# zhexin1904/gtsam_personal

Hardware: AMD Instinct MI355X
Metric: LM iterations/sec (higher is better)
Workload: dtype f64; 1 GPU; synthetic BAL 1000 cameras / 100000 points / 1000002 factors (GeneralSFMFactor<Cal3Bundler> + 2 priors), seed 42, METIS ordering (Ordering::Metis of the reference, fixture-carried permutation), LM legacy defaults; ordering=metis, cameras=1000, points=100000, factors=1000002, fronts=100001, parallelism=single GPU

## Files before the change

### gtsam_personal_amd/csrc/kernels_dense.hpp

```cpp
#pragma once
#include <hip/hip_runtime.h>

#include <type_traits>

#include "kernels_front.hpp"

namespace lmgpu {

typedef double double4_t __attribute__((ext_vector_type(4)));

struct RowSrc {
  int32_t idx;
  int32_t i;
};
__device__ __forceinline__ void assemble_row_body(const FrontDesc& F, int64_t f_off, int ld, const int32_t* __restrict__ rowptr, const RowSrc* __restrict__ src,
                                                  const ChildRef* __restrict__ childs, const int32_t* __restrict__ cmap,
                                                  const FrontFac* __restrict__ ffac, const FacDesc* __restrict__ fd, double* __restrict__ pool,
                                                  int R, bool with_factors) {
  const int lane = threadIdx.x & 63;
  double* Arow = pool + f_off + (size_t)R * ld;
  for (int e = rowptr[R]; e < rowptr[R + 1]; e++) {
    const RowSrc sr = src[e];
    if (sr.idx >= 0) {
      const ChildRef c = childs[sr.idx];
// ... 449 lines not shown
__global__ __launch_bounds__(256) void hbm_backsolve_dataflow_kernel(FrontDesc F, int64_t f_off, int ld, const int32_t* __restrict__ fxoff,
                                                                      const double* __restrict__ pool, const double* __restrict__ inv,
                                                                      const double* __restrict__ y, double* __restrict__ xbuf,
                                                                      unsigned int* __restrict__ flags, double* __restrict__ delta,
                                                                      int* __restrict__ status) {
  __shared__ double acc[NB];
  __shared__ double xs[NB];
  __shared__ int ok, s_ticket;
  const int nblk = gridDim.x;
  if (threadIdx.x == 0) s_ticket = (int)atomicAdd(&flags[nblk], 1u);
  __syncthreads();
  const int b = nblk - 1 - s_ticket;
  const int r0 = b * NB, nb = min(NB, F.nf - r0);
  const int tid = threadIdx.x, row = tid >> 2, quarter = tid & 3;
  const double* A = pool + f_off;
  if (tid < NB) acc[tid] = (tid < nb) ? y[r0 + tid] : 0.0;
  if (tid == 0) ok = 1;
  __syncthreads();
  const double* arow = A + (size_t)(r0 + row) * ld;
  double ibv[16];
  {
    const double* ib = inv + (size_t)b * NB * NB + row * NB + quarter * 16;
#pragma unroll
    for (int k = 0; k < 16; k++) ibv[k] = ib[k];
  }
  auto load_rv = [&](int j, double(&r)[16]) {
    const int c0 = j * NB, ncol = min(NB, F.nf - c0);
#pragma unroll
    for (int k = 0; k < 16; k++) {
      const int c = quarter * 16 + k;
      r[k] = (j > b && row < nb && c < ncol) ? arow[c0 + c] : 0.0;
    }
  };
  double rv[16], rv_next[16];
  load_rv(nblk - 1, rv);
  for (int j = nblk - 1; j > b; j--) {
    const int c0 = j * NB, ncol = min(NB, F.nf - c0);
    if (tid < NB) {
      double v = 0.0;
      if (tid < ncol) {
        long spins = 0;
        for (;;) {
          v = __hip_atomic_load(&xbuf[c0 + tid], __ATOMIC_RELAXED, __HIP_MEMORY_SCOPE_AGENT);
          if (__double_as_longlong(v) != -1LL) break;
          __builtin_amdgcn_s_sleep(1);
          if (++spins > 2000000L) {
            ok = 0;
            v = 0.0;
            break;
          }
        }
      }
      xs[tid] = v;
    }
    load_rv(j - 1, rv_next);
    __syncthreads();
    if (!ok) break;
    double s = 0;
#pragma unroll
    for (int k = 0; k < 16; k++) s += rv[k] * xs[quarter * 16 + k];
    s += __shfl_xor(s, 1);
    s += __shfl_xor(s, 2);
    if (quarter == 0) acc[row] -= s;
#pragma unroll
    for (int k = 0; k < 16; k++) rv[k] = rv_next[k];
    __syncthreads();
  }
  if (!ok) {
    if (tid == 0) atomicExch(status + 1, 1 + F.id);
  }
  double s = 0;
#pragma unroll
  for (int k = 0; k < 16; k++) s += ibv[k] * acc[quarter * 16 + k];
  s += __shfl_xor(s, 1);
  s += __shfl_xor(s, 2);
  if (quarter == 0 && row < nb) {
    const double pub = (s != s) ? __longlong_as_double(0x7ff8000000000000LL) : s;
    __hip_atomic_store(&xbuf[r0 + row], pub, __ATOMIC_RELAXED, __HIP_MEMORY_SCOPE_AGENT);
    delta[fxoff[F.fx_begin + r0 + row]] = s;
    if (s != s) atomicMin(status, F.id);
  }
}

__global__ __launch_bounds__(256) void hbm_backsolve_dataflow2_kernel(FrontDesc F, int64_t f_off, int ld, const int32_t* __restrict__ fxoff,
                                                                       const double* __restrict__ pool, const double* __restrict__ inv16,
                                                                       const double* __restrict__ y ,
                                                                       double* __restrict__ xbuf, unsigned int* __restrict__ flags,
                                                                       double* __restrict__ delta, int* __restrict__ status) {
  typedef double d4_t __attribute__((ext_vector_type(4)));
  constexpr int NB = 64;
  __shared__ double Rl[64][65];
  __shared__ double Xl[64][65];
  __shared__ double Ml[64][65];
  __shared__ double Il[4][16][17];
  __shared__ double acc[NB], xs[NB], ub[NB];
  __shared__ int ok, s_ticket;
  const int nblk = gridDim.x;
  if (threadIdx.x == 0) s_ticket = (int)atomicAdd(&flags[nblk], 1u);
  __syncthreads();
  const int b = nblk - 1 - s_ticket;
  const int r0 = b * NB, nb = min(NB, F.nf - r0);
  const int tid = threadIdx.x, row = tid >> 2, quarter = tid & 3, lane = tid & 63, wave = tid >> 6;
  const int kk = lane >> 4, cc = lane & 15;
  const double* A = pool + f_off;
  const int n = F.n;
  if (tid < NB) acc[tid] = (tid < nb) ? (y ? y[r0 + tid] : A[(size_t)(r0 + tid) * ld + n - 1]) : 0.0;
  if (tid == 0) ok = 1;
  for (int idx = tid; idx < 64 * 64; idx += 256) {
    const int p = idx >> 6, q = idx & 63;
    double v = (p == q) ? 1.0 : 0.0;
    if (p < nb && q < nb && q >= p) v = A[(size_t)(r0 + p) * ld + r0 + q];
    Rl[p][q] = v;
    Xl[p][q] = 0.0;
  }
  const double* I16 = inv16 + (size_t)(b >> 2) * 4096 + (size_t)(4 * (b & 3)) * 256;
  for (int idx = tid; idx < 4 * 256; idx += 256) Il[idx >> 8][(idx >> 4) & 15][idx & 15] = I16[idx];
  __syncthreads();
  if (wave == 0) {
#pragma unroll
    for (int h = 0; h < 4; h++) {
#pragma unroll
      for (int r = 0; r < 4; r++) Xl[16 * h + kk + 4 * r][16 * h + cc] = Il[h][kk + 4 * r][cc];
      __builtin_amdgcn_wave_barrier();
      asm volatile("s_waitcnt lgkmcnt(0)" ::: "memory");
#pragma unroll
      for (int g = h - 1; g >= 0; g--) {
        d4_t m = d4_t{0, 0, 0, 0};
#pragma unroll
        for (int k = g + 1; k <= h; k++)
#pragma unroll
          for (int r = 0; r < 4; r++) m = __builtin_amdgcn_mfma_f64_16x16x4f64(Rl[16 * g + cc][16 * k + 4 * r + kk], Xl[16 * k + 4 * r + kk][16 * h + cc], m, 0, 0, 0);
        d4_t x = d4_t{0, 0, 0, 0};
#pragma unroll
        for (int r = 0; r < 4; r++) x = __builtin_amdgcn_mfma_f64_16x16x4f64(-Il[g][cc][4 * r + kk], m[r], x, 0, 0, 0);
#pragma unroll
        for (int r = 0; r < 4; r++) Xl[16 * g + kk + 4 * r][16 * h + cc] = x[r];
        __builtin_amdgcn_wave_barrier();
        asm volatile("s_waitcnt lgkmcnt(0)" ::: "memory");
      }
    }
  }
  __syncthreads();
  if (b + 1 < nblk) {
    const int c0n = (b + 1) * NB, ncoln = min(NB, F.nf - c0n);
    for (int idx = tid; idx < 64 * 64; idx += 256) {
      const int p = idx >> 6, q = idx & 63;
      Rl[p][q] = (p < nb && q < ncoln) ? A[(size_t)(r0 + p) * ld + c0n + q] : 0.0;
    }
    __syncthreads();
#pragma unroll
    for (int h = 0; h < 4; h++) {
      d4_t m = d4_t{0, 0, 0, 0};
#pragma unroll
      for (int k = 0; k < 16; k++) m = __builtin_amdgcn_mfma_f64_16x16x4f64(Xl[16 * wave + cc][4 * k + kk], Rl[4 * k + kk][16 * h + cc], m, 0, 0, 0);
#pragma unroll
      for (int r = 0; r < 4; r++) Ml[16 * wave + kk + 4 * r][16 * h + cc] = m[r];
    }
  }
  __syncthreads();
  double ibv[16], mv[16];
#pragma unroll
  for (int k = 0; k < 16; k++) {
    ibv[k] = Xl[row][quarter * 16 + k];
    mv[k] = Ml[row][quarter * 16 + k];
  }
  const double* arow = A + (size_t)(r0 + row) * ld;
  auto load_rv = [&](int j, double(&r)[16]) {
    const int c0 = j * NB, ncol = min(NB, F.nf - c0);
#pragma unroll
    for (int k = 0; k < 16; k++) {
      const int c = quarter * 16 + k;
      r[k] = (j > b + 1 && row < nb && c < ncol) ? arow[c0 + c] : 0.0;
    }
  };
  auto poll = [&](int j) {
    const int c0 = j * NB, ncol = min(NB, F.nf - c0);
    if (tid < NB) {
      double v = 0.0;
      if (tid < ncol) {
        long spins = 0;
        for (;;) {
          v = __hip_atomic_load(&xbuf[c0 + tid], __ATOMIC_RELAXED, __HIP_MEMORY_SCOPE_AGENT);
          if (__double_as_longlong(v) != -1LL) break;
          __builtin_amdgcn_s_sleep(1);
          if (++spins > 2000000L) {
            ok = 0;
            v = 0.0;
            break;
          }
        }
      }
      xs[tid] = v;
    }
  };
  double rv[16], rv_next[16];
  load_rv(nblk - 1, rv);
  for (int j = nblk - 1; j > b + 1; j--) {
    poll(j);
    load_rv(j - 1, rv_next);
    __syncthreads();
    if (!ok) break;
    double s = 0;
#pragma unroll
    for (int k = 0; k < 16; k++) s += rv[k] * xs[quarter * 16 + k];
    s += __shfl_xor(s, 1);
    s += __shfl_xor(s, 2);
    if (quarter == 0) acc[row] -= s;
#pragma unroll
    for (int k = 0; k < 16; k++) rv[k] = rv_next[k];
    __syncthreads();
  }
  {
    double s = 0;
#pragma unroll
    for (int k = 0; k < 16; k++) s += ibv[k] * acc[quarter * 16 + k];
    s += __shfl_xor(s, 1);
    s += __shfl_xor(s, 2);
    if (quarter == 0) ub[row] = s;
  }
  double xr;
  if (b + 1 < nblk && ok) {
    poll(b + 1);
    __syncthreads();
    double s = 0;
#pragma unroll
    for (int k = 0; k < 16; k++) s += mv[k] * xs[quarter * 16 + k];
    s += __shfl_xor(s, 1);
    s += __shfl_xor(s, 2);
    xr = ub[row] - s;
  } else {
    __syncthreads();
    xr = ub[row];
  }
  if (!ok && tid == 0) atomicExch(status + 1, 1 + F.id);
  if (quarter == 0 && row < nb) {
    const double pub = (xr != xr) ? __longlong_as_double(0x7ff8000000000000LL) : xr;
    __hip_atomic_store(&xbuf[r0 + row], pub, __ATOMIC_RELAXED, __HIP_MEMORY_SCOPE_AGENT);
    delta[fxoff[F.fx_begin + r0 + row]] = xr;
    if (xr != xr) atomicMin(status, F.id);
  }
}

}
```

### gtsam_personal_amd/csrc/lmgpu.hip

```cpp
#include <hip/hip_runtime.h>
#include <rccl/rccl.h>

#include <algorithm>
#include <chrono>
#include <cmath>
#include <cstdio>
#include <cstdlib>
#include <cstring>
#include <condition_variable>
#include <limits>
#include <mutex>
#include <string>
#include <map>
#include <vector>

#include "../../include/lmgpu.h"
#include "kernels_dense.hpp"
#include "kernels_potrf.hpp"
#include "kernels_step.hpp"
#include "dense_schedule.hpp"
#include "kernels_batched.hpp"
#include "kernels_level.hpp"
#include "kernels_bayes.hpp"
#include "kernels_schur.hpp"
// ... 947 lines not shown
  if (h->cfg.world_size > 1) HIPCHECK(hipMemsetAsync(h->delta, 0, h->ntot * sizeof(double), s));
  const bool merge = h->merge_backsub && h->cfg.world_size == 1 && !(h->cfg.flags & LMGPU_FLAG_SPLIT_ROOT);
  const bool no_bsd_runs = dev_switch("LMGPU_NO_BSD_RUNS") != nullptr;
  const int NFR = (int)h->h_fronts.size();
  if (h->n_fill_backsub < 0 || h->fill_backsub_merge != (int)merge) {
    std::vector<FillChunk> fills;
    if (merge) {
      add_fill(fills, h->d_bs_done, (size_t)(NFR + h->levels.size() + 1) * sizeof(unsigned int), 0u);
      add_fill(fills, h->delta, h->ntot * sizeof(double), 0xffffffffu);
    }
    if (h->bsd_x_count > 0) {
      add_fill(fills, h->d_bsd_x, h->bsd_x_count * sizeof(double), 0xffffffffu);
      add_fill(fills, h->d_bsd_ticket, h->levels.size() * sizeof(unsigned int), 0u);
    }
    if (h->d_fill_backsub) {
      HIPCHECK(hipStreamSynchronize(s));
      (void)hipFree(h->d_fill_backsub);
      h->d_fill_backsub = nullptr;
    }
    h->n_fill_backsub = (int)fills.size();
    h->fill_backsub_merge = (int)merge;
    if (!fills.empty()) {
      const int rcu = upload(h, &h->d_fill_backsub, fills);
      if (rcu) return rcu;
    }
  }
  if (h->n_fill_backsub > 0) hipLaunchKernelGGL(fill_chunks_kernel, dim3(h->n_fill_backsub), dim3(256), 0, s, (const FillChunk*)h->d_fill_backsub);
  int seg_hi = -1, seg_lo = -1;
  auto run_level = [&](const LevelWork& L) {
    if (L.lds_nf_max > LDSB_SMALL_NF) {
      hipLaunchKernelGGL(lds_backsub_wide_kernel, dim3(L.list_count), dim3(256), (size_t)(L.lds_rsd_max + LDSB_TAIL) * sizeof(double), s,
                         (const int32_t*)(h->d_lists + L.list_begin), L.list_count, (const FrontDesc*)h->d_fronts, (const int32_t*)h->d_fxoff,
                         (const int32_t*)h->d_sxoff, (const double*)h->pool, h->delta, h->d_status);
    } else {
      hipLaunchKernelGGL(lds_backsub_kernel, dim3((L.list_count + 3) / 4), dim3(256), 0, s, (const int32_t*)(h->d_lists + L.list_begin),
                         L.list_count, (const FrontDesc*)h->d_fronts, (const int32_t*)h->d_fxoff, (const int32_t*)h->d_sxoff,
                         (const double*)h->pool, h->delta, h->d_status);
    }
  };
  auto flush_segment = [&]() -> int {
    if (seg_hi < 0) return LMGPU_OK;
    const int kt = h->kt.begin(LMGPU_KT_BACKSUB_LDS, s);
    if (seg_hi == seg_lo) {
      run_level(h->levels[seg_hi]);
    } else {
      const int b = h->levels[seg_lo].list_begin, e = h->levels[seg_hi].list_begin + h->levels[seg_hi].list_count;
      int rsdmax = 0;
      for (int l = seg_lo; l <= seg_hi; l++) rsdmax = std::max(rsdmax, h->levels[l].lds_rsd_max);
      hipLaunchKernelGGL(lds_backsub_merged_kernel, dim3(e - b), dim3(256), (size_t)(rsdmax + LDSB_TAIL) * sizeof(double), s, (const int32_t*)h->d_lists, b, e,
                         (const FrontDesc*)h->d_fronts, (const int32_t*)h->d_fxoff, (const int32_t*)h->d_sxoff, (const double*)h->pool, h->delta,
                         h->d_status, (const int32_t*)h->d_bs_parent, (const int32_t*)h->d_bs_pos, h->d_bs_done, h->d_bs_done + NFR + seg_hi);
    }
    h->kt.end(kt, s);
    seg_hi = seg_lo = -1;
    return LMGPU_OK;
  };
  for (int li = (int)h->levels.size() - 1; li >= 0; li--) {
    const LevelWork& L = h->levels[li];
    if (merge && !L.hbm.empty()) {
      const int rcf = flush_segment();
      if (rcf) return rcf;
    }
    const int brun = (merge && !h->bsd_run_of.empty() && !no_bsd_runs) ? h->bsd_run_of[li] : -1;
    if (brun >= 0) {
      const lmgpu_handle::BsdRun& R = h->bsd_runs[brun];
      const int kt = h->kt.begin(LMGPU_KT_BACKSUB_HBM, s);
      hipLaunchKernelGGL(hbm_backsolve_blocks_kernel, dim3(R.count), dim3(256), 0, s, (const BsdBlock*)(h->d_bsd_run_table + R.begin), h->d_bsd_ticket + li,
                         (const int32_t*)h->d_fxoff, (const int32_t*)h->d_sxoff, (const double*)h->pool, h->delta, h->d_bsd_x, h->d_status, 1);
      h->kt.end(kt, s);
    }
    if (L.bsd_count > 0 && brun == -1) {
      const int kt = h->kt.begin(LMGPU_KT_BACKSUB_HBM, s);
      hipLaunchKernelGGL(hbm_backsolve_blocks_kernel, dim3(L.bsd_count), dim3(256), 0, s, (const BsdBlock*)(h->d_bsd_table + L.bsd_begin),
                         (L.bsd_count <= h->num_cus && !h->bsd_ticket) ? (unsigned int*)nullptr : h->d_bsd_ticket + li, (const int32_t*)h->d_fxoff,
                         (const int32_t*)h->d_sxoff, (const double*)h->pool, h->delta, h->d_bsd_x, h->d_status);
      h->kt.end(kt, s);
    }
    for (int fi : L.hbm) {
      const FrontDesc& F = h->h_fronts[fi];
      if (F.nf <= BSS_MAX_NF) continue;
      const int64_t off = h->f_off[fi];
      const int ld = h->f_ld[fi];
      const int kt = h->kt.begin(LMGPU_KT_BACKSUB_HBM, s);
      const int nblk = (F.nf + NB - 1) / NB;
      const bool has_sep = F.n - F.nf - 1 > 0;
      if (has_sep)
        hipLaunchKernelGGL(hbm_rhs_init_kernel, dim3(F.nf), dim3(64), 0, s, F, off, ld, (const int32_t*)h->d_sxoff, (const double*)h->pool,
                           (const double*)h->delta, h->ywork);
      HIPCHECK(hipMemsetAsync(h->bs_flags, 0, (nblk + 1) * sizeof(unsigned int), s));
      HIPCHECK(hipMemsetAsync(h->bs_x, 0xff, (size_t)nblk * NB * sizeof(double), s));
      if (h->inv16_owner == fi && !dev_switch("LMGPU_NO_INV16_REUSE")) {
        hipLaunchKernelGGL(hbm_backsolve_dataflow2_kernel, dim3(nblk), dim3(256), 0, s, F, off, ld, (const int32_t*)h->d_fxoff, (const double*)h->pool,
                           (const double*)h->inv16, has_sep ? (const double*)h->ywork : (const double*)nullptr, h->bs_x, h->bs_flags, h->delta,
                           h->d_status);
      } else {
        if (!has_sep)
          hipLaunchKernelGGL(hbm_rhs_init_kernel, dim3(F.nf), dim3(64), 0, s, F, off, ld, (const int32_t*)h->d_sxoff, (const double*)h->pool,
                             (const double*)h->delta, h->ywork);
        hipLaunchKernelGGL((hbm_invert_diag_kernel<NB>), dim3(nblk), dim3(NB), 0, s, (const double*)(h->pool + off), ld, F.nf, h->bs_inv);
        hipLaunchKernelGGL((hbm_backsolve_dataflow_kernel<NB>), dim3(nblk), dim3(256), 0, s, F, off, ld, (const int32_t*)h->d_fxoff,
                           (const double*)h->pool, (const double*)h->bs_inv, (const double*)h->ywork, h->bs_x, h->bs_flags, h->delta,
                           h->d_status);
      }
      h->kt.end(kt, s);
    }
    if (merge) {
      if (L.list_count > 0) {
        if (seg_hi < 0) seg_hi = li;
        seg_lo = li;
      }
      if (li == 0 || !h->levels[li - 1].hbm.empty()) {
        const int rcf = flush_segment();
        if (rcf) return rcf;
      }
    } else if (L.list_count > 0) {
      const int kt = h->kt.begin(LMGPU_KT_BACKSUB_LDS, s);
      run_level(L);
      h->kt.end(kt, s);
    }
  }
  HIPCHECK(hipGetLastError());
  return LMGPU_OK;
}

__global__ void set_scalar_kernel(double* p, double v) { *p = v; }


int pcg_ensure(lmgpu_handle* h) {
  if (h->pcg_ready) return LMGPU_OK;
  const Plan& P = h->plan;
  std::vector<int32_t> xo(P.xoff.begin(), P.xoff.begin() + P.n_vars + 1);
  std::vector<int64_t> loff(P.n_vars);
  int64_t lsz = 0;
  for (int s = 0; s < P.n_vars; s++) {
    loff[s] = lsz;
    lsz += (int64_t)P.dims[s] * P.dims[s];
  }
  std::vector<FacDesc> fd(h->nfac);
  HIPCHECK(hipMemcpy(fd.data(), h->d_fd, fd.size() * sizeof(FacDesc), hipMemcpyDeviceToHost));
  std::vector<int64_t> yoff(h->nfac);
  int64_t ysz = 0;
  for (int f = 0; f < h->nfac; f++) {
    yoff[f] = ysz;
    ysz += fd[f].rows;
  }
  int rc;
  if ((rc = upload(h, &h->pcg_xoff, xo))) return rc;
  if ((rc = upload(h, &h->pcg_loff, loff))) return rc;
  if ((rc = upload(h, &h->pcg_yoff, yoff))) return rc;
  const size_t n = std::max(1, h->ntot);
  HIPCHECK(hipMalloc((void**)&h->pcg_H, std::max<int64_t>(1, lsz) * sizeof(double)));
  HIPCHECK(hipMalloc((void**)&h->pcg_L, std::max<int64_t>(1, lsz) * sizeof(double)));
  HIPCHECK(hipMalloc((void**)&h->pcg_rhs, n * sizeof(double)));
  HIPCHECK(hipMalloc((void**)&h->pcg_r, n * sizeof(double)));
  HIPCHECK(hipMalloc((void**)&h->pcg_p, n * sizeof(double)));
  HIPCHECK(hipMalloc((void**)&h->pcg_q, n * sizeof(double)));
  HIPCHECK(hipMalloc((void**)&h->pcg_y, std::max<int64_t>(1, ysz) * sizeof(double)));
  HIPCHECK(hipMalloc((void**)&h->pcg_part, 3 * PCG_MAXPART * sizeof(double)));
  HIPCHECK(hipMalloc((void**)&h->pcg_ctl, sizeof(PcgCtl)));
  HIPCHECK(hipHostMalloc((void**)&h->h_pcg_ctl, sizeof(PcgCtl), hipHostMallocDefault));
  HIPCHECK(hipHostMalloc((void**)&h->h_pcg_done, sizeof(int32_t), hipHostMallocDefault));
  for (int i = 0; i < 3; i++) HIPCHECK(hipEventCreate(&h->pcg_ev[i]));
  h->pcg_ready = true;
  return LMGPU_OK;
}

__global__ void pcg_reset_ctl_kernel(PcgCtl* c) {
  c->status = 0x7fffffff;
  c->iters = 0;
}

int pcg_solve_enqueue(lmgpu_handle* h, double lambda) {
  int rc = pcg_ensure(h);
  if (rc) return rc;
  const lmgpu_pcg_params& pp = h->pcgp;
  if (pp.maxIterations + 1 > h->pcg_cap) {
    if (h->pcg_gam) (void)hipFree(h->pcg_gam);
// ... 1478 lines not shown
        const FrontDesc& F = h->h_fronts[fi];
        const lmgpu_handle::GatherRange& G = h->gather[fi];
        if (fr.nf > NBO || (F.pad & 1) || G.leaf_count > 0 || G.pblk_short + G.pblk_long + G.vblk_count > 0 || dev_switch("LMGPU_NO_MED")) continue;
        med.push_back(fi);
        h->is_med[fi] = 1;
        L.med_max_fac = std::max(L.med_max_fac, F.fac_count);
        L.med_max_child = std::max(L.med_max_child, F.child_count);
        L.med_max_nf = std::max(L.med_max_nf, fr.nf);
        L.med_max_cols = std::max(L.med_max_cols, fr.n - fr.nf);
        L.med_max_n = std::max(L.med_max_n, (int)fr.n);
      }
      L.med_count = (int)med.size() - L.med_begin;
      max_med = std::max(max_med, L.med_count);
    }
    if ((rc = upload(h, &h->d_med_list, med))) return rc;
    if (max_med > 0) HIPCHECK(hipMalloc((void**)&h->inv16_med, (size_t)max_med * 16 * 256 * sizeof(double)));
    if ((rc = upload(h, &h->d_f_off, h->f_off))) return rc;
    if ((rc = upload(h, &h->d_f_ld, h->f_ld))) return rc;
  }
  if ((rc = upload(h, &h->d_row_begin, h->row_begin))) return rc;
  {
    std::vector<MedFront> mfs;
    for (const LevelWork& L : h->levels)
      for (int fi : L.hbm)
        if (h->is_med[fi]) mfs.push_back(MedFront{h->h_fronts[fi], h->f_off[fi], h->f_ld[fi], h->row_begin[fi]});
    if ((rc = upload(h, &h->d_med_fronts, mfs))) return rc;
    h->fuse_levels = (int)h->levels.size() >= 12 && h->cfg.world_size == 1;
    if (const char* e = dev_switch("LMGPU_FUSE_LEVELS")) h->fuse_levels = atoi(e) != 0 && h->cfg.world_size == 1;
    std::vector<LevelTask> tasks;
    int li = 0;
    for (LevelWork& L : h->levels) {
      const int l = li++;
      L.fuse_task_count = 0;
      int nmax, jcap, threads;
      if (!h->fuse_levels || L.med_count == 0 || !(L.med_max_fac > 0 || L.med_max_child > 0)) continue;
      if (h->merge_elim && h->elim_seg_of[l] != -1) continue;
      if (!level_lds_class(h, l, &nmax, &jcap, &threads)) continue;
      L.fuse_task_begin = (int)tasks.size();
      L.fuse_nmax = nmax;
      L.fuse_jcap = jcap;
      L.fuse_threads = 256;
      if (const char* e = dev_switch("LMGPU_FUSE_THREADS")) L.fuse_threads = atoi(e) == 1024 && threads == 1024 ? 1024 : 256;
      for (int q = 0; q < L.list_count; q++) tasks.push_back(LevelTask{0, L.list_begin + q, 0, 0});
      for (int m = 0; m < L.med_count; m++) {
        const FrontDesc& F = mfs[L.med_begin + m].F;
        for (int r = 0; r < F.n; r += 4) tasks.push_back(LevelTask{1, m, r, 0});
      }
      for (int m = 0; m < L.med_count; m++) tasks.push_back(LevelTask{2, m, 0, 0});
      for (int m = 0; m < L.med_count; m++) {
        const FrontDesc& F = mfs[L.med_begin + m].F;
        for (int st = 0; st * 64 < F.n - F.nf; st++) tasks.push_back(LevelTask{3, m, st, 0});
      }
      for (int m = 0; m < L.med_count; m++) {
        const FrontDesc& F = mfs[L.med_begin + m].F;
        const int S = (F.n - F.nf + 63) / 64;
        for (int sj = 0; sj < S; sj++)
          for (int si = 0; si <= sj; si++)
            for (int qd = 0; qd < 4; qd++) tasks.push_back(LevelTask{4, m, si | (sj << 8), qd});
      }
      L.fuse_task_count = (int)tasks.size() - L.fuse_task_begin;
    }
    if (!tasks.empty()) {
      if ((rc = upload(h, &h->d_level_tasks, tasks))) return rc;
      h->n_level_sync = (int)mfs.size();
      HIPCHECK(hipMalloc((void**)&h->d_level_sync, std::max<size_t>(1, mfs.size()) * sizeof(LevelSync)));
    } else {
      h->fuse_levels = false;
    }
  }
  if ((rc = upload(h, &h->d_rowptr, rowptr))) return rc;
  if ((rc = upload(h, &h->d_rowsrc, rowsrc))) return rc;
  if ((rc = upload(h, &h->d_gpblk, gpblk))) return rc;
  if ((rc = upload(h, &h->d_gzero, gzero))) return rc;
  if ((rc = upload(h, &h->d_gpent, gpent))) return rc;
  if ((rc = upload(h, &h->d_gvblk, gvblk))) return rc;
  if ((rc = upload(h, &h->d_gvent, gvent))) return rc;
  HIPCHECK(hipMalloc((void**)&h->d_gcorner, std::max<size_t>(1, (size_t)n_gleaf) * sizeof(double)));
  if ((rc = finalize_vectors(h))) return rc;
  {
    int max_nf = 1;
    for (int fi = 0; fi < NF; fi++)
      if (h->front_active[fi] && P.fronts[fi].cls == 1) max_nf = std::max(max_nf, P.fronts[fi].nf);
    const int max_blk = (max_nf + NB - 1) / NB;
    HIPCHECK(hipMalloc((void**)&h->bs_inv, (size_t)max_blk * NB * NB * sizeof(double)));
    HIPCHECK(hipMalloc((void**)&h->inv16, (size_t)((P.max_front_n + NBO - 1) / NBO + 2) * 16 * 256 * sizeof(double)));
    h->pflags_panels = (P.max_front_n + NBO - 1) / NBO + 1;
    HIPCHECK(hipMalloc((void**)&h->d_pflags, (size_t)h->pflags_panels * PDF_FLAG_WORDS * sizeof(unsigned int)));

    HIPCHECK(hipMalloc((void**)&h->bs_x, (size_t)max_blk * NB * sizeof(double)));
    HIPCHECK(hipMalloc((void**)&h->bs_flags, (size_t)(max_blk + 1) * sizeof(unsigned int)));
  }
  return LMGPU_OK;
}

int lmgpu_total_dim(const lmgpu_handle* h) { return (h && h->finalized) ? h->ntot : -1; }
int lmgpu_total_store(const lmgpu_handle* h) { return (h && h->finalized) ? h->nstore : -1; }

int lmgpu_set_values(lmgpu_handle* h, const double* packed) {
  if (!h) return LMGPU_INVALID;
  if (!h->finalized || !packed) {
    h->err = "lmgpu_set_values: refused (!h->finalized || !packed)";
    return LMGPU_INVALID;
  }
  int rc = need_device(h);
  if (rc) return rc;
  const Plan& P = h->plan;
  for (int t = 0; t < kNumVarTypes; t++) {
    if (P.type_count[t] == 0) continue;
    std::vector<double> buf((size_t)P.type_count[t] * kVarStore[t]);
    for (int s = 0; s < P.n_vars; s++)
      if (P.types[s] == t) std::memcpy(&buf[(size_t)P.tidx[s] * kVarStore[t]], packed + P.voff[s], kVarStore[t] * sizeof(double));
    HIPCHECK(hipMemcpy(h->vals[h->cur][t], buf.data(), buf.size() * sizeof(double), hipMemcpyHostToDevice));
  }
  h->have_values = true;
  return LMGPU_OK;
}

int lmgpu_get_values(lmgpu_handle* h, double* packed) {
  if (!h) return LMGPU_INVALID;
  if (!h->finalized || !packed || !h->have_values) {
    h->err = "lmgpu_get_values: refused (!h->finalized || !packed || !h->have_values)";
    return LMGPU_INVALID;
  }
  int rc = need_device(h);
  if (rc) return rc;
  const Plan& P = h->plan;
  HIPCHECK(hipStreamSynchronize(h->stream));
  for (int t = 0; t < kNumVarTypes; t++) {
    if (P.type_count[t] == 0) continue;
    std::vector<double> buf((size_t)P.type_count[t] * kVarStore[t]);
    HIPCHECK(hipMemcpy(buf.data(), h->vals[h->cur][t], buf.size() * sizeof(double), hipMemcpyDeviceToHost));
    for (int s = 0; s < P.n_vars; s++)
      if (P.types[s] == t) std::memcpy(packed + P.voff[s], &buf[(size_t)P.tidx[s] * kVarStore[t]], kVarStore[t] * sizeof(double));
  }
  return LMGPU_OK;
}

int lmgpu_save_values(lmgpu_handle* h) {
  if (!h) return LMGPU_INVALID;
  if (!h->finalized || !h->have_values) {
    h->err = "lmgpu_save_values: refused (!h->finalized || !h->have_values)";
    return LMGPU_INVALID;
  }
  int rc = need_device(h);
  if (rc) return rc;
  for (int t = 0; t < kNumVarTypes; t++) {
    const size_t bytes = std::max<size_t>(1, (size_t)h->plan.type_count[t] * kVarStore[t]) * sizeof(double);
    if (!h->saved[t]) HIPCHECK(hipMalloc((void**)&h->saved[t], bytes));
    HIPCHECK(hipMemcpyAsync(h->saved[t], h->vals[h->cur][t], bytes, hipMemcpyDeviceToDevice, h->stream));
  }
  HIPCHECK(hipStreamSynchronize(h->stream));
  return LMGPU_OK;
}

int lmgpu_restore_values(lmgpu_handle* h) {
  if (!h) return LMGPU_INVALID;
  if (!h->finalized || !h->saved[0]) {
    h->err = "lmgpu_restore_values: refused (!h->finalized || !h->saved[0])";
    return LMGPU_INVALID;
  }
  int rc = need_device(h);
  if (rc) return rc;
  for (int t = 0; t < kNumVarTypes; t++) {
    const size_t bytes = std::max<size_t>(1, (size_t)h->plan.type_count[t] * kVarStore[t]) * sizeof(double);
    HIPCHECK(hipMemcpyAsync(h->vals[h->cur][t], h->saved[t], bytes, hipMemcpyDeviceToDevice, h->stream));
  }
  return LMGPU_OK;
}

int lmgpu_error(lmgpu_handle* h, double* total) {
  if (!h) return LMGPU_INVALID;
  if (!h->finalized || !total || !h->have_values) {
// ... 1217 lines not shown
```

Measured before the change: 131.2 LM iterations/s.

## Add wide 128-row dataflow back-solve kernel for large HBM fronts

Replaces the 64-row-per-block dataflow back-substitution for large fronts with a 512-thread kernel that handles 128-row blocks. Each block inverts its two 64x64 diagonal sub-blocks with MFMA from reused inv16 inverses, precomputes the product with the next block's off-diagonal coupling and parks it in scratch, and then streams the remaining tiles with double-buffered loads while polling for upstream solutions. The aim is to halve the length of the serial dependency chain and take the coupling GEMV off the critical path. The cost is more registers and shared memory per block and a spin-limit fallback. The old kernel is now compiled only under test hooks.

```diff
diff --git a/gtsam_personal_amd/csrc/kernels_dense.hpp b/gtsam_personal_amd/csrc/kernels_dense.hpp
--- a/gtsam_personal_amd/csrc/kernels_dense.hpp
+++ b/gtsam_personal_amd/csrc/kernels_dense.hpp
@@ -555,11 +555,14 @@
   }
 }
 
+#ifdef LMGPU_TEST_HOOKS
+template <bool STAMP = false>
 __global__ __launch_bounds__(256) void hbm_backsolve_dataflow2_kernel(FrontDesc F, int64_t f_off, int ld, const int32_t* __restrict__ fxoff,
                                                                        const double* __restrict__ pool, const double* __restrict__ inv16,
                                                                        const double* __restrict__ y ,
                                                                        double* __restrict__ xbuf, unsigned int* __restrict__ flags,
-                                                                       double* __restrict__ delta, int* __restrict__ status) {
+                                                                       double* __restrict__ delta, int* __restrict__ status,
+                                                                       unsigned long long* __restrict__ stamps = nullptr) {
   typedef double d4_t __attribute__((ext_vector_type(4)));
   constexpr int NB = 64;
   __shared__ double Rl[64][65];
@@ -575,6 +578,7 @@
   const int r0 = b * NB, nb = min(NB, F.nf - r0);
   const int tid = threadIdx.x, row = tid >> 2, quarter = tid & 3, lane = tid & 63, wave = tid >> 6;
   const int kk = lane >> 4, cc = lane & 15;
+  if (STAMP && tid == 0) stamps[3 * b] = wall_clock64();
   const double* A = pool + f_off;
   const int n = F.n;
   if (tid < NB) acc[tid] = (tid < nb) ? (y ? y[r0 + tid] : A[(size_t)(r0 + tid) * ld + n - 1]) : 0.0;
@@ -694,6 +698,7 @@
   double xr;
   if (b + 1 < nblk && ok) {
     poll(b + 1);
+    if (STAMP && tid == 0) stamps[3 * b + 1] = wall_clock64();
     __syncthreads();
     double s = 0;
 #pragma unroll
@@ -712,6 +717,298 @@
     delta[fxoff[F.fx_begin + r0 + row]] = xr;
     if (xr != xr) atomicMin(status, F.id);
   }
-}
-
-}
+  if (STAMP && tid == 0) stamps[3 * b + 2] = wall_clock64();
+}
+#endif
+
+__device__ __forceinline__ void bsw_invert64(const double (*Rl)[65], double (*Xl)[65], const double (*Il)[16][17], int kk, int cc) {
+  typedef double d4_t __attribute__((ext_vector_type(4)));
+#pragma unroll
+  for (int h = 0; h < 4; h++) {
+#pragma unroll
+    for (int r = 0; r < 4; r++) Xl[16 * h + kk + 4 * r][16 * h + cc] = Il[h][kk + 4 * r][cc];
+    __builtin_amdgcn_wave_barrier();
+    asm volatile("s_waitcnt lgkmcnt(0)" ::: "memory");
+#pragma unroll
+    for (int g = h - 1; g >= 0; g--) {
+      d4_t m = d4_t{0, 0, 0, 0};
+#pragma unroll
+      for (int k = g + 1; k <= h; k++)
+#pragma unroll
+        for (int r = 0; r < 4; r++) m = __builtin_amdgcn_mfma_f64_16x16x4f64(Rl[16 * g + cc][16 * k + 4 * r + kk], Xl[16 * k + 4 * r + kk][16 * h + cc], m, 0, 0, 0);
+      d4_t x = d4_t{0, 0, 0, 0};
+#pragma unroll
+      for (int r = 0; r < 4; r++) x = __builtin_amdgcn_mfma_f64_16x16x4f64(-Il[g][cc][4 * r + kk], m[r], x, 0, 0, 0);
+#pragma unroll
+      for (int r = 0; r < 4; r++) Xl[16 * g + kk + 4 * r][16 * h + cc] = x[r];
+      __builtin_amdgcn_wave_barrier();
+      asm volatile("s_waitcnt lgkmcnt(0)" ::: "memory");
+    }
+  }
+}
+
+#define BSW_NB 128
+#define BSW_SPIN_LIMIT 2000000L
+template <bool STAMP = false>
+__global__ __launch_bounds__(512) void hbm_backsolve_wide_kernel(FrontDesc F, int64_t f_off, int ld, const int32_t* __restrict__ fxoff,
+                                                                  const double* __restrict__ pool, const double* __restrict__ inv16,
+                                                                  const double* __restrict__ y ,
+                                                                  double* __restrict__ xbuf, unsigned int* __restrict__ flags,
+                                                                  double* __restrict__ delta, int* __restrict__ status,
+                                                                  double* mpark ,
+                                                                  unsigned long long* __restrict__ stamps = nullptr) {
+  typedef double d4_t __attribute__((ext_vector_type(4)));
+  constexpr int NB = BSW_NB;
+  __shared__ double T[4][64][65];
+  __shared__ double Il[8][16][17];
+  __shared__ double rhs[NB], ub[NB];
+  __shared__ double xs[8][NB];
+  __shared__ int s_ticket;
+  const int nblk = gridDim.x;
+  if (threadIdx.x == 0) s_ticket = (int)atomicAdd(&flags[nblk], 1u);
+  __syncthreads();
+  const int b = nblk - 1 - s_ticket;
+  const int nf = F.nf, n = F.n;
+  const int r0 = b * NB, nb = min(NB, nf - r0);
+  const int tid = threadIdx.x, lane = tid & 63, wave = __builtin_amdgcn_readfirstlane(tid >> 6);
+  const int kk = lane >> 4, cc = lane & 15;
+  const double* A = pool + f_off;
+  if (STAMP && tid == 0) stamps[3 * b] = wall_clock64();
+  const int myslot = ((lane >> 5) & 1) * 8 + ((lane >> 4) & 1) * 4 + ((lane >> 3) & 1) * 2 + ((lane >> 2) & 1);
+  const int frow = 16 * wave + myslot;
+  const int frc = min(r0 + frow, nf - 1);
+  const double yv = y ? y[frc] : A[(size_t)frc * ld + n - 1];
+  const int hr = 2 * ((cc >> 3) & 1) + ((cc >> 2) & 1);
+  const int prow = 16 * wave + kk + 4 * hr;
+  const int po = fxoff[F.fx_begin + min(r0 + prow, nf - 1)];
+  const bool has_next = b + 1 < nblk;
+  const int c0n = (b + 1) * NB, ncoln = has_next ? min(NB, nf - c0n) : 0;
+  double g11[8], g22[8], g12[8], gn[2][2][8];
+#pragma unroll
+  for (int i = 0; i < 8; i++) {
+    const int p = wave + 8 * i, q = lane;
+    const double e = (p == q) ? 1.0 : 0.0;
+    g11[i] = (p < nb && q < nb && q >= p) ? A[(size_t)(r0 + p) * ld + r0 + q] : e;
+    g22[i] = (64 + p < nb && 64 + q < nb && q >= p) ? A[(size_t)(r0 + 64 + p) * ld + r0 + 64 + q] : e;
+    g12[i] = (p < nb && 64 + q < nb) ? A[(size_t)(r0 + p) * ld + r0 + 64 + q] : 0.0;
+#pragma unroll
+    for (int kh = 0; kh < 2; kh++)
+#pragma unroll
+      for (int ch = 0; ch < 2; ch++)
+        gn[kh][ch][i] = (64 * kh + p < nb && 64 * ch + q < ncoln) ? A[(size_t)(r0 + 64 * kh + p) * ld + c0n + 64 * ch + q] : 0.0;
+  }
+#pragma unroll
+  for (int i = 0; i < 8; i++) {
+    const int p = wave + 8 * i, q = lane;
+    T[0][p][q] = g11[i];
+    T[1][p][q] = g22[i];
+    T[2][p][q] = 0.0;
+    T[3][p][q] = 0.0;
+  }
+  const double* I16 = inv16 + (size_t)(b >> 1) * 4096 + (size_t)(8 * (b & 1)) * 256;
+  for (int idx = tid; idx < 8 * 256; idx += 512) {
+    const int h = idx >> 8, i = (idx >> 4) & 15, j = idx & 15;
+    Il[h][i][j] = (16 * h < nb) ? I16[idx] : ((i == j) ? 1.0 : 0.0);
+  }
+  __syncthreads();
+  if (wave < 2) bsw_invert64(T[wave], T[2 + wave], Il + 4 * wave, kk, cc);
+  __syncthreads();
+#pragma unroll
+  for (int i = 0; i < 8; i++) T[0][wave + 8 * i][lane] = g12[i];
+  __syncthreads();
+  {
+    const int ti = wave >> 1;
+#pragma unroll
+    for (int u = 0; u < 2; u++) {
+      const int tj = 2 * (wave & 1) + u;
+      d4_t m = d4_t{0, 0, 0, 0};
+#pragma unroll
+      for (int k = 0; k < 16; k++) m = __builtin_amdgcn_mfma_f64_16x16x4f64(T[0][16 * ti + cc][4 * k + kk], T[3][4 * k + kk][16 * tj + cc], m, 0, 0, 0);
+#pragma unroll
+      for (int r = 0; r < 4; r++) T[1][16 * ti + kk + 4 * r][16 * tj + cc] = m[r];
+    }
+    __syncthreads();
+#pragma unroll
+    for (int u = 0; u < 2; u++) {
+      const int tj = 2 * (wave & 1) + u;
+      d4_t m = d4_t{0, 0, 0, 0};
+#pragma unroll
+      for (int k = 0; k < 16; k++) m = __builtin_amdgcn_mfma_f64_16x16x4f64(-T[2][16 * ti + cc][4 * k + kk], T[1][4 * k + kk][16 * tj + cc], m, 0, 0, 0);
+#pragma unroll
+      for (int r = 0; r < 4; r++) T[0][16 * ti + kk + 4 * r][16 * tj + cc] = m[r];
+    }
+    __syncthreads();
+  }
+  d4_t mB[8];
+#pragma unroll
+  for (int h = 0; h < 8; h++) mB[h] = d4_t{0, 0, 0, 0};
+  if (has_next) {
+#pragma unroll
+    for (int kh = 0; kh < 2; kh++) {
+#pragma unroll
+      for (int ch = 0; ch < 2; ch++) {
+#pragma unroll
+        for (int i = 0; i < 8; i++) T[1][wave + 8 * i][lane] = gn[kh][ch][i];
+        __syncthreads();
+        if (wave < 4 || kh == 1) {
+          const double(*Xop)[65] = (wave >= 4) ? T[3] : (kh == 0 ? T[2] : T[0]);
+          const int xr0 = 16 * (wave & 3);
+#pragma unroll
+          for (int hh = 0; hh < 4; hh++)
+#pragma unroll
+            for (int k = 0; k < 16; k++)
+              mB[4 * ch + hh] = __builtin_amdgcn_mfma_f64_16x16x4f64(Xop[xr0 + cc][4 * k + kk], T[1][4 * k + kk][16 * hh + cc], mB[4 * ch + hh], 0, 0, 0);
+        }
+        __syncthreads();
+      }
+    }
+  }
+  double* Mp = mpark + (size_t)b * NB * NB + tid;
+  if (has_next) {
+#pragma unroll
+    for (int h = 0; h < 8; h++)
+#pragma unroll
+      for (int r = 0; r < 4; r++) Mp[(4 * h + r) * 512] = mB[h][r];
+  }
+  auto load_tile = [&](int j, double(&t)[32]) {
+    const bool real = j > b + 1, parked = j == b + 1 && has_next;
+    const double* base = real ? A + (size_t)(r0 + 16 * wave) * ld : (parked ? mpark + (size_t)b * NB * NB : A + (size_t)r0 * ld);
+    const int stride = real ? ld : (parked ? 1024 : 0);
+    const int o0 = real ? min(NB * j + lane, nf - 1) : (parked ? tid : r0), o1 = real ? min(NB * j + 64 + lane, nf - 1) : (parked ? tid + 512 : r0);
+#pragma unroll
+    for (int k = 0; k < 16; k++) {
+      const double* row = base + (size_t)k * stride;
+      t[2 * k] = row[o0];
+      t[2 * k + 1] = row[o1];
+    }
+  };
+  bool dead = false;
+  auto poll2 = [&](int j, double& x0, double& x1) {
+    long spins = 0;
+    for (;;) {
+      x0 = __hip_atomic_load(&xbuf[NB * j + lane], __ATOMIC_RELAXED, __HIP_MEMORY_SCOPE_AGENT);
+      x1 = __hip_atomic_load(&xbuf[NB * j + 64 + lane], __ATOMIC_RELAXED, __HIP_MEMORY_SCOPE_AGENT);
+      if (__double_as_longlong(x0) != -1LL && __double_as_longlong(x1) != -1LL) break;
+      if (dead || ++spins > BSW_SPIN_LIMIT) {
+        dead = true;
+        x0 = x1 = 0.0;
+        break;
+      }
+      __builtin_amdgcn_s_sleep(1);
+    }
+  };
+  auto look = [&](int j, double& x0, double& x1) {
+    x0 = __hip_atomic_load(&xbuf[NB * j + lane], __ATOMIC_RELAXED, __HIP_MEMORY_SCOPE_AGENT);
+    x1 = __hip_atomic_load(&xbuf[NB * j + 64 + lane], __ATOMIC_RELAXED, __HIP_MEMORY_SCOPE_AGENT);
+  };
+  double acc[16], ta[32], tb[32], e0, e1;
+#pragma unroll
+  for (int k = 0; k < 16; k++) acc[k] = 0.0;
+  look(nblk - 1, e0, e1);
+  __builtin_amdgcn_sched_barrier(0);
+  load_tile(nblk - 1, ta);
+  __builtin_amdgcn_sched_barrier(0);
+  load_tile(nblk - 2, tb);
+  __builtin_amdgcn_sched_barrier(0);
+  auto fold = [&](int j, double(&t)[32]) {
+    double x0 = e0, x1 = e1;
+    if (__double_as_longlong(x0) == -1LL || __double_as_longlong(x1) == -1LL) poll2(j, x0, x1);
+    look(j - 1, e0, e1);
+    __builtin_amdgcn_sched_barrier(0);
+#pragma unroll
+    for (int k = 0; k < 16; k++) acc[k] = fma(t[2 * k + 1], x1, fma(t[2 * k], x0, acc[k]));
+    __builtin_amdgcn_sched_barrier(0);
+    load_tile(j - 2, t);
+    __builtin_amdgcn_sched_barrier(0);
+  };
+  {
+    int j = nblk - 1;
+    for (; j - 1 > b + 1; j -= 2) {
+      fold(j, ta);
+      fold(j - 1, tb);
+    }
+    if (j > b + 1) fold(j, ta);
+  }
+  {
+    int slot;
+    const double tot = wave_reduce_slots<16>(acc, lane, slot);
+    if ((lane & 3) == 0) rhs[frow] = (frow < nb) ? yv - tot : 0.0;
+    __syncthreads();
+    const int row = tid >> 2, q = tid & 3;
+    double s0 = 0, s1 = 0, s2 = 0, s3 = 0;
+    if (row < 64) {
+      const double* xr = (q < 2) ? &T[2][row][32 * q] : &T[0][row][32 * (q - 2)];
+      const double* rr = rhs + 32 * q;
+#pragma unroll
+      for (int k = 0; k < 32; k += 4) {
+        s0 = fma(xr[k], rr[k], s0);
+        s1 = fma(xr[k + 1], rr[k + 1], s1);
+        s2 = fma(xr[k + 2], rr[k + 2], s2);
+        s3 = fma(xr[k + 3], rr[k + 3], s3);
+      }
+    } else {
+      const double* xr = &T[3][row - 64][16 * q];
+      const double* rr = rhs + 64 + 16 * q;
+#pragma unroll
+      for (int k = 0; k < 16; k += 4) {
+        s0 = fma(xr[k], rr[k], s0);
+        s1 = fma(xr[k + 1], rr[k + 1], s1);
+        s2 = fma(xr[k + 2], rr[k + 2], s2);
+        s3 = fma(xr[k + 3], rr[k + 3], s3);
+      }
+    }
+    double s = (s0 + s1) + (s2 + s3);
+    s += __shfl_xor(s, 1);
+    s += __shfl_xor(s, 2);
+    if (q == 0) ub[row] = s;
+    __syncthreads();
+  }
+  double xr = ub[prow];
+  if (has_next) {
+    double x0 = e0, x1 = e1;
+    if (__double_as_longlong(x0) == -1LL || __double_as_longlong(x1) == -1LL) poll2(b + 1, x0, x1);
+    if (STAMP && tid == 0) stamps[3 * b + 1] = wall_clock64();
+    xs[wave][lane] = x0;
+    xs[wave][64 + lane] = x1;
+    __builtin_amdgcn_wave_barrier();
+    asm volatile("s_waitcnt lgkmcnt(0)" ::: "memory");
+    double sa[4], sb[4];
+#pragma unroll
+    for (int r = 0; r < 4; r++) sa[r] = sb[r] = 0.0;
+    auto sums = [&](const double(&mv)[32]) {
+#pragma unroll
+      for (int h = 0; h < 8; h += 2) {
+        const double xa = xs[wave][16 * h + cc], xc = xs[wave][16 * h + 16 + cc];
+#pragma unroll
+        for (int r = 0; r < 4; r++) {
+          sa[r] = fma(mv[4 * h + r], xa, sa[r]);
+          sb[r] = fma(mv[4 * h + 4 + r], xc, sb[r]);
+        }
+      }
+    };
+    if (((nblk - b) & 1) == 0)
+      sums(ta);
+    else
+      sums(tb);
+#pragma unroll
+    for (int r = 0; r < 4; r++) sa[r] += sb[r];
+    const bool h8 = (cc & 8) != 0, h4 = (cc & 4) != 0;
+    const double k0 = h8 ? sa[2] : sa[0], k1 = h8 ? sa[3] : sa[1], d0 = h8 ? sa[0] : sa[2], d1 = h8 ? sa[1] : sa[3];
+    const double t0 = k0 + __shfl_xor(d0, 8), t1 = k1 + __shfl_xor(d1, 8);
+    double v = (h4 ? t1 : t0) + __shfl_xor(h4 ? t0 : t1, 4);
+    v += __shfl_xor(v, 2);
+    v += __shfl_xor(v, 1);
+    xr -= v;
+  }
+  if ((cc & 3) == 0) {
+    const double pub = (prow < nb) ? ((xr != xr) ? __longlong_as_double(0x7ff8000000000000LL) : xr) : 0.0;
+    __hip_atomic_store(&xbuf[r0 + prow], pub, __ATOMIC_RELAXED, __HIP_MEMORY_SCOPE_AGENT);
+    if (prow < nb) {
+      delta[po] = xr;
+      if (xr != xr) atomicMin(status, F.id);
+    }
+  }
+  if (STAMP && tid == 0) stamps[3 * b + 2] = wall_clock64();
+  if (__any(dead) && lane == 0) atomicExch(status + 1, 1 + F.id);
+}
+}
diff --git a/gtsam_personal_amd/csrc/lmgpu.hip b/gtsam_personal_amd/csrc/lmgpu.hip
--- a/gtsam_personal_amd/csrc/lmgpu.hip
+++ b/gtsam_personal_amd/csrc/lmgpu.hip
@@ -1053,17 +1053,25 @@
       const int64_t off = h->f_off[fi];
       const int ld = h->f_ld[fi];
       const int kt = h->kt.begin(LMGPU_KT_BACKSUB_HBM, s);
-      const int nblk = (F.nf + NB - 1) / NB;
       const bool has_sep = F.n - F.nf - 1 > 0;
       if (has_sep)
         hipLaunchKernelGGL(hbm_rhs_init_kernel, dim3(F.nf), dim3(64), 0, s, F, off, ld, (const int32_t*)h->d_sxoff, (const double*)h->pool,
                            (const double*)h->delta, h->ywork);
+      const bool reuse = h->inv16_owner == fi && !dev_switch("LMGPU_NO_INV16_REUSE");
+      const bool wide = reuse && !dev_switch("LMGPU_BACKSOLVE_HOP64");
+      const int bw = wide ? BSW_NB : NB, nblk = (F.nf + bw - 1) / bw;
       HIPCHECK(hipMemsetAsync(h->bs_flags, 0, (nblk + 1) * sizeof(unsigned int), s));
-      HIPCHECK(hipMemsetAsync(h->bs_x, 0xff, (size_t)nblk * NB * sizeof(double), s));
-      if (h->inv16_owner == fi && !dev_switch("LMGPU_NO_INV16_REUSE")) {
-        hipLaunchKernelGGL(hbm_backsolve_dataflow2_kernel, dim3(nblk), dim3(256), 0, s, F, off, ld, (const int32_t*)h->d_fxoff, (const double*)h->pool,
+      HIPCHECK(hipMemsetAsync(h->bs_x, 0xff, (size_t)nblk * bw * sizeof(double), s));
+      if (wide) {
+        hipLaunchKernelGGL((hbm_backsolve_wide_kernel<false>), dim3(nblk), dim3(512), 0, s, F, off, ld, (const int32_t*)h->d_fxoff, (const double*)h->pool,
                            (const double*)h->inv16, has_sep ? (const double*)h->ywork : (const double*)nullptr, h->bs_x, h->bs_flags, h->delta,
-                           h->d_status);
+                           h->d_status, h->bs_inv, (unsigned long long*)nullptr);
+#ifdef LMGPU_TEST_HOOKS
+      } else if (reuse) {
+        hipLaunchKernelGGL((hbm_backsolve_dataflow2_kernel<false>), dim3(nblk), dim3(256), 0, s, F, off, ld, (const int32_t*)h->d_fxoff, (const double*)h->pool,
+                           (const double*)h->inv16, has_sep ? (const double*)h->ywork : (const double*)nullptr, h->bs_x, h->bs_flags, h->delta,
+                           h->d_status, (unsigned long long*)nullptr);
+#endif
       } else {
         if (!has_sep)
           hipLaunchKernelGGL(hbm_rhs_init_kernel, dim3(F.nf), dim3(64), 0, s, F, off, ld, (const int32_t*)h->d_sxoff, (const double*)h->pool,
@@ -2708,12 +2716,12 @@
     for (int fi = 0; fi < NF; fi++)
       if (h->front_active[fi] && P.fronts[fi].cls == 1) max_nf = std::max(max_nf, P.fronts[fi].nf);
     const int max_blk = (max_nf + NB - 1) / NB;
-    HIPCHECK(hipMalloc((void**)&h->bs_inv, (size_t)max_blk * NB * NB * sizeof(double)));
+    HIPCHECK(hipMalloc((void**)&h->bs_inv, (size_t)((max_nf + BSW_NB - 1) / BSW_NB) * BSW_NB * BSW_NB * sizeof(double)));
     HIPCHECK(hipMalloc((void**)&h->inv16, (size_t)((P.max_front_n + NBO - 1) / NBO + 2) * 16 * 256 * sizeof(double)));
     h->pflags_panels = (P.max_front_n + NBO - 1) / NBO + 1;
     HIPCHECK(hipMalloc((void**)&h->d_pflags, (size_t)h->pflags_panels * PDF_FLAG_WORDS * sizeof(unsigned int)));
 
-    HIPCHECK(hipMalloc((void**)&h->bs_x, (size_t)max_blk * NB * sizeof(double)));
+    HIPCHECK(hipMalloc((void**)&h->bs_x, (size_t)((max_nf + BSW_NB - 1) / BSW_NB) * BSW_NB * sizeof(double)));
     HIPCHECK(hipMalloc((void**)&h->bs_flags, (size_t)(max_blk + 1) * sizeof(unsigned int)));
   }
   return LMGPU_OK;
```

After: 133.1 LM iterations/s (median of 6 runs). 1.01x the previous value.
